# Senpai-sama06/real-time-audio-visual-zooming

Measured on AMD Instinct MI355X. Metric: beamformed TF-bins/sec (2-ch, 1024-pt STFT) + SIR dB delta vs reference, higher is better.
Workload: dtype f32

## Files before the change

### include/avz.h

```cpp
#ifndef AVZ_H_
#define AVZ_H_

#ifdef __cplusplus
extern "C" {
#endif

#define AVZ_OK 0
#define AVZ_ERR_ARG (-1)
#define AVZ_ERR_SHAPE (-2)
#define AVZ_ERR_HIP (-3)
#define AVZ_ERR_UNSUPPORTED (-4)
#define AVZ_ERR_ALIGN (-5)

#define AVZ_MASK_IBM 0
#define AVZ_MASK_IPD 1
#define AVZ_MASK_EXTERNAL 2
#define AVZ_MASK_ONES 3

#define AVZ_PF_NONE 0
#define AVZ_PF_IBM_TARGET 1
#define AVZ_PF_EXT_FLOOR 2
#define AVZ_PF_EXT_MUL 3
#define AVZ_PF_IRM 4

// ... 74 lines not shown
  int batch;
  int frames;
  const float* Y;
  long long y_stride_b, y_stride_m, y_stride_f;
  const float* mask;
  long long mask_stride_b, mask_stride_f;
  const double* steer;
  float* S;
  long long s_stride_b, s_stride_f;
  double* cov_out;
  float* w_out;
  int* fallback;
} avz_spectral_args;
int avz_beamform_spectral(const avz_plan* plan, const avz_spectral_args* args, void* hip_stream);

int avz_istft(const avz_plan* plan, int batch, int frames, const float* S, long long s_stride_b,
              long long s_stride_f, float* out, long long out_stride, float* peak,
              void* workspace, long long workspace_bytes, void* hip_stream);

int avz_plan_set_timing(avz_plan* plan, int enable);
int avz_plan_set_timing_period(avz_plan* plan, int period);
int avz_plan_get_timing(avz_plan* plan, double* ms_avg , int* calls);
int avz_plan_set_ibm_stats(avz_plan* plan, unsigned long long* counts);
int avz_plan_set_diagnostics(avz_plan* plan, int synth_variant, int ipf_mode);
int avz_ibm_window(int n, float* out);

int avz_stft(const avz_plan* plan, int batch, int channels, const int* len, int max_len,
             const float* x, long long x_stride, long long ch_stride, float* Y,
             long long y_stride_b, long long y_stride_c, long long y_stride_f,
             void* hip_stream);

int avz_chunk_split(int n_items, int channels, int chunk, const int* item_utt,
                    const int* item_start, const int* len, const float* x, long long x_stride,
                    long long x_ch_stride, float* items, long long item_stride,
                    long long item_ch_stride, void* hip_stream);

int avz_chunk_merge(int batch, int max_len, int hop, int item_out_len, const int* len,
                    const int* item_base, const float* item_out, long long item_out_stride,
                    float* y, long long y_stride, float* peak, int normalize, double norm_eps,
                    void* hip_stream);

#define AVZ_FEAT_LOGMAG_IPD 1
#define AVZ_FEAT_TFLITE 2
int avz_mask_features(const avz_plan* plan, int layout, int batch, const int* len, int max_len,
                      const float* x, long long x_stride, long long ch_stride, float* feat,
                      long long s_b, long long s_c, long long s_f, long long s_t,
// ... 40 lines not shown
```

### real-time-audio-visual-zooming_amd/avz/_lib.py

```python
from __future__ import annotations

import ctypes as ct
import os

import torch

_HERE = os.path.dirname(os.path.abspath(__file__))
LIB_PATH = os.environ.get("AVZ_LIB", os.path.join(_HERE, "libavz.so"))

AVZ_OK = 0
AVZ_ERR_ARG = -1
AVZ_ERR_SHAPE = -2
AVZ_ERR_HIP = -3
AVZ_ERR_UNSUPPORTED = -4
AVZ_ERR_ALIGN = -5

MASK_IBM, MASK_IPD, MASK_EXTERNAL, MASK_ONES = 0, 1, 2, 3
PF_NONE, PF_IBM_TARGET, PF_EXT_FLOOR, PF_EXT_MUL, PF_IRM = 0, 1, 2, 3, 4
FALLBACK_MIC0, FALLBACK_MEAN, FALLBACK_BATCH = 0, 1, 2
NORM_NONE, NORM_PEAK = 0, 1
BF_MVDR, BF_HYBRID_NULL = 0, 1
FEAT_LOGMAG_IPD, FEAT_TFLITE = 1, 2

EXPORTED = [
    "avz_plan_create", "avz_plan_destroy", "avz_plan_get_config", "avz_num_frames",
    "avz_mvdr_batch", "avz_plan_set_timing", "avz_plan_get_timing", "avz_stft",
    "avz_plan_set_timing_period",
    "avz_chunk_split", "avz_chunk_merge", "avz_mask_features", "avz_srp_scan",
    "avz_projection_metrics", "avz_scene_workspace_bytes", "avz_scene_mix", "avz_strerror",
    "avz_last_hip_error", "avz_version", "avz_mvdr_workspace_bytes",
    "avz_mvdr_covariance", "avz_solve_covariance", "avz_apply_istft", "avz_beamform_spectral",
    "avz_istft", "avz_scene_generate_workspace_bytes", "avz_scene_generate",
    "avz_projection_metrics_scaled", "avz_plan_set_ibm_stats", "avz_plan_set_diagnostics",
    "avz_ibm_window",
]


class AvzConfig(ct.Structure):
    _fields_ = [
        ("fs", ct.c_int), ("n_fft", ct.c_int), ("hop", ct.c_int),
        ("sigma", ct.c_double), ("angle_deg", ct.c_double), ("mic_d", ct.c_double),
        ("c_sound", ct.c_double), ("fmin_hz", ct.c_double),
        ("mask_mode", ct.c_int), ("postfilter", ct.c_int),
        ("pf_floor", ct.c_double), ("weight_eps", ct.c_double),
        ("normalize", ct.c_int), ("norm_eps", ct.c_double),
        ("max_batch", ct.c_int), ("max_samples", ct.c_int),
        ("beamformer", ct.c_int), ("bypass_hz", ct.c_double), ("cond_max", ct.c_double),
        ("singular_fallback", ct.c_int), ("ibm_kappa", ct.c_double),
    ]


class AvzBatchArgs(ct.Structure):
    _fields_ = [
        ("batch", ct.c_int), ("len", ct.c_void_p), ("max_len", ct.c_int),
        ("mix", ct.c_void_p), ("mix_stride", ct.c_longlong), ("ch_stride", ct.c_longlong),
        ("ref_tgt", ct.c_void_p), ("ref_int", ct.c_void_p), ("ref_stride", ct.c_longlong),
        ("ext_mask", ct.c_void_p), ("mask_stride_b", ct.c_longlong),
# ... 48 lines not shown
    lib.avz_plan_create.argtypes = [ct.POINTER(P), ct.POINTER(AvzConfig)]
    lib.avz_plan_destroy.argtypes = [P]
    lib.avz_plan_get_config.argtypes = [P, ct.POINTER(AvzConfig)]
    lib.avz_num_frames.argtypes = [P, ct.c_int]
    lib.avz_mvdr_batch.argtypes = [P, ct.POINTER(AvzBatchArgs), P]
    lib.avz_mvdr_workspace_bytes.argtypes = [P, ct.c_int, ct.c_int]
    lib.avz_mvdr_workspace_bytes.restype = ct.c_longlong
    lib.avz_mvdr_covariance.argtypes = [P, ct.POINTER(AvzBatchArgs), P]
    lib.avz_solve_covariance.argtypes = [P, ct.c_int, P, P, P, P, P]
    lib.avz_apply_istft.argtypes = [P, ct.POINTER(AvzBatchArgs), P, P]
    lib.avz_beamform_spectral.argtypes = [P, ct.POINTER(AvzSpectralArgs), P]
    lib.avz_istft.argtypes = [P, ct.c_int, ct.c_int, P, ct.c_longlong, ct.c_longlong, P,
                              ct.c_longlong, P, P, ct.c_longlong, P]
    for name in ("avz_mvdr_covariance", "avz_solve_covariance", "avz_apply_istft",
                 "avz_beamform_spectral", "avz_istft"):
        getattr(lib, name).restype = ct.c_int
    lib.avz_stft.argtypes = [P, ct.c_int, ct.c_int, P, ct.c_int, P, ct.c_longlong, ct.c_longlong,
                             P, ct.c_longlong, ct.c_longlong, ct.c_longlong, P]
    I, LL = ct.c_int, ct.c_longlong
    lib.avz_plan_set_timing.argtypes = [P, I]
    lib.avz_plan_set_timing_period.argtypes = [P, I]
    lib.avz_plan_get_timing.argtypes = [P, ct.POINTER(ct.c_double), ct.POINTER(I)]
    lib.avz_plan_set_ibm_stats.argtypes = [P, P]
    lib.avz_plan_set_diagnostics.argtypes = [P, I, I]
    lib.avz_ibm_window.argtypes = [I, ct.POINTER(ct.c_float)]
    lib.avz_chunk_split.argtypes = [I, I, I, P, P, P, P, LL, LL, P, LL, LL, P]
    lib.avz_chunk_merge.argtypes = [I, I, I, I, P, P, P, LL, P, LL, P, I, ct.c_double, P]
    lib.avz_mask_features.argtypes = [P, I, I, P, I, P, LL, LL, P, LL, LL, LL, LL, P]
    D = ct.c_double
    lib.avz_srp_scan.argtypes = [P, I, P, I, P, LL, LL, I, D, D, D, D, P, P]
    lib.avz_projection_metrics.argtypes = [I, I, P, P, LL, P, LL, P, LL, P, P, P]
    lib.avz_projection_metrics_scaled.argtypes = [I, I, P, P, LL, P, D, P, LL, P, LL, P, P, P]
    lib.avz_scene_workspace_bytes.argtypes = [I, I, I]
    lib.avz_scene_workspace_bytes.restype = LL
    lib.avz_scene_mix.argtypes = [I, I, I, P, P, P, D, D, D, D, D, P, LL, LL, P, P, LL, P, LL, P]
    lib.avz_scene_generate_workspace_bytes.argtypes = [I, I, I]
    lib.avz_scene_generate_workspace_bytes.restype = LL
    lib.avz_scene_generate.argtypes = [I, LL, I, I, ct.c_uint, D, D, D, D, D, P, LL, LL, P, P, LL,
                                       P, LL, P]
    lib.avz_strerror.argtypes = [ct.c_int]
    lib.avz_strerror.restype = ct.c_char_p
    lib.avz_last_hip_error.restype = ct.c_char_p
    for name in ("avz_plan_create", "avz_plan_destroy", "avz_plan_get_config", "avz_num_frames",
                 "avz_mvdr_batch", "avz_stft", "avz_chunk_split", "avz_chunk_merge",
                 "avz_plan_set_timing", "avz_plan_get_timing", "avz_mask_features",
                 "avz_plan_set_timing_period",
                 "avz_srp_scan", "avz_projection_metrics", "avz_scene_mix",
                 "avz_scene_generate", "avz_projection_metrics_scaled", "avz_version",
                 "avz_plan_set_ibm_stats", "avz_plan_set_diagnostics", "avz_ibm_window"):
        getattr(lib, name).restype = ct.c_int
    if lib.avz_version() != ABI_VERSION:
        raise ImportError(f"libavz ABI version {lib.avz_version()} != {ABI_VERSION} "
                          "(AvzBatchArgs / AvzSpectralArgs layouts); rebuild")
    return lib


lib = _load()


def check(rc: int, what: str) -> int:
    if rc < 0:
        msg = lib.avz_strerror(rc).decode()
        if rc == AVZ_ERR_HIP:
            msg += ": " + lib.avz_last_hip_error().decode()
        raise AvzError(f"{what} failed ({rc}): {msg}")
    return rc
```

### real-time-audio-visual-zooming_amd/avz/engine.py

```python
from __future__ import annotations

import ctypes as ct
from dataclasses import dataclass, field

import torch

from . import _lib
from ._lib import AvzBatchArgs, AvzConfig, check, lib

MASKS = {"ibm": _lib.MASK_IBM, "ipd": _lib.MASK_IPD, "external": _lib.MASK_EXTERNAL,
         "ones": _lib.MASK_ONES}
POSTFILTERS = {"none": _lib.PF_NONE, "ibm": _lib.PF_IBM_TARGET, "floor": _lib.PF_EXT_FLOOR,
               "mul": _lib.PF_EXT_MUL, "irm": _lib.PF_IRM}
FALLBACKS = {"mic0": _lib.FALLBACK_MIC0, "mean": _lib.FALLBACK_MEAN,
             "batch": _lib.FALLBACK_BATCH}
NORMS = {"none": _lib.NORM_NONE, "peak": _lib.NORM_PEAK}
BEAMFORMERS = {"mvdr": _lib.BF_MVDR, "hybrid_null": _lib.BF_HYBRID_NULL}


def n_frames(length: int, hop: int) -> int:
    return -(-length // hop) + 1


def out_length(length: int, hop: int) -> int:
# ... 61 lines not shown
        self._h = h
        self.hop = cfg.n_fft // 2
        self.F = cfg.n_fft // 2 + 1

    def __del__(self):
        h = getattr(self, "_h", None)
        if h is not None and h.value:
            lib.avz_plan_destroy(h)
            self._h = None

    KERNELS = ("analysis", "solve", "synthesis", "finalize")

    def set_timing(self, enable: bool = True, analysis_only: bool = False,
                   period: int = 1) -> None:
        mode = (2 if analysis_only else 1) if enable else 0
        check(lib.avz_plan_set_timing_period(self._h, int(period)), "avz_plan_set_timing_period")
        check(lib.avz_plan_set_timing(self._h, mode), "avz_plan_set_timing")

    def set_ibm_stats(self, counts) -> None:
        if counts is not None:
            assert counts.dtype == torch.int64 and counts.is_cuda and counts.numel() >= 2
        check(lib.avz_plan_set_ibm_stats(self._h, _ptr(counts)), "avz_plan_set_ibm_stats")
        self._ibm_stats = counts

    def set_diagnostics(self, synth_variant: int = 2, ipf_mode: int = 0) -> None:
        check(lib.avz_plan_set_diagnostics(self._h, int(synth_variant), int(ipf_mode)),
              "avz_plan_set_diagnostics")

    def timing(self) -> dict:
        ms = (ct.c_double * 4)()
        n = ct.c_int()
        check(lib.avz_plan_get_timing(self._h, ms, ct.byref(n)), "avz_plan_get_timing")
        return {"calls": n.value, **{k: ms[i] for i, k in enumerate(self.KERNELS)}}

    def frames(self, length: int) -> int:
        return check(lib.avz_num_frames(self._h, int(length)), "avz_num_frames")

    def out_len(self, length: int) -> int:
        return out_length(length, self.hop)

    def alloc_out(self, batch: int, max_len: int, device) -> torch.Tensor:
        n = self.out_len(max_len)
        return torch.empty((batch, (n + 3) // 4 * 4), dtype=torch.float32, device=device)

    def workspace_bytes(self, batch: int, max_len: int) -> int:
        return check(lib.avz_mvdr_workspace_bytes(self._h, int(batch), int(max_len)),
# ... 268 lines not shown
```

### real-time-audio-visual-zooming_amd/csrc/avz_capi.cpp

```cpp
#include <hip/hip_runtime.h>

#include <algorithm>
#include <cmath>
#include <complex>
#include <limits>
#include <cstdlib>
#include <cstring>
#include <new>
#include <string>
#include <vector>

#include "../../include/avz.h"
#include "avz_internal.h"

struct Workspace {
  float* part;
  uint32_t* mwords;
  float* coef;
  float* heads;
  float* tails;
  uint32_t* peak_u;
  int* flag;
  float* pf_gain;
  float* tpart;
// ... 58 lines not shown
    w->xpend = units ? reinterpret_cast<uint32_t*>(q) : nullptr; q += sz_xp;
    w->xdfr = units ? reinterpret_cast<uint32_t*>(q) : nullptr; q += sz_xd;
    w->xunc = units ? reinterpret_cast<uint32_t*>(q) : nullptr; q += sz_xu;
    w->xst = units ? reinterpret_cast<uint32_t*>(q) : nullptr; q += sz_xs;
    w->xst_bytes = sz_xs;
    w->xst_units = units;
    w->xres = units ? reinterpret_cast<float*>(q) : nullptr; q += sz_xr;
  }
  return sz_part + sz_mw + sz_coef + 2 * sz_ht + 6 * sz_b + sz_gain + sz_tpart + 2 * sz_seam +
         sz_xp + sz_xd + sz_xu + sz_xs + sz_xr;
}

struct avz_plan {
  avz_config cfg;
  double tau1, tau2;
  int max_frames;
  int nchunk;
  void* arena;
  double* steer;
  double* xtw;
  float* xwin;
  float ibm_cert;
  unsigned long long* xstat;
  int synth_variant;
  int dbg_ipf;
  Workspace ws;
  bool timing;
  int n_k;
  hipEvent_t ev[2][8];
  bool ev_pending[2];
  int ev_kern[2];
  int ev_next;
  int period;
  long long seen;
  double ms_sum[4];
  int ms_calls;
};

static void timing_drain(avz_plan* p, int set) {
  if (!p->ev_pending[set]) return;
  p->ev_pending[set] = false;
  int last = 0;
  for (int i = 0; i < p->n_k; ++i)
    if ((p->ev_kern[set] >> i) & 1) last = i;
  if (hipEventSynchronize(p->ev[set][2 * last + 1]) != hipSuccess) return;
  for (int i = 0; i < p->n_k; ++i) {
// ... 100 lines not shown
    const size_t sz_tab = sz_steer + sz_xtw + sz_xwin;
    const size_t sz_ws = ws_layout(c, c.max_batch, p->nchunk, nullptr, nullptr);
    hipError_t e = hipMalloc(&p->arena, sz_tab + sz_ws);
    if (e != hipSuccess) {
      delete p;
      return hip_fail(e);
    }
    char* q = static_cast<char*>(p->arena);
    p->steer = reinterpret_cast<double*>(q);
    p->xtw = reinterpret_cast<double*>(q + sz_steer);
    p->xwin = reinterpret_cast<float*>(q + sz_steer + sz_xtw);
    ws_layout(c, c.max_batch, p->nchunk, q + sz_tab, &p->ws);
    if (p->ws.xst) {
      e = hipMemset(p->ws.xst, 0, p->ws.xst_bytes);
      if (e != hipSuccess) {
        (void)hipFree(p->arena);
        delete p;
        return hip_fail(e);
      }
    }
    const double kappa = c.ibm_kappa == 0.0 ? AVZ_IBM_KAPPA : c.ibm_kappa;
    p->ibm_cert = kappa > 0.0 ? (float)(kappa * 0x1p-24) : 0.0f;
    p->xstat = nullptr;
    p->synth_variant = 2;
    p->dbg_ipf = 0;
    std::vector<double> xt((size_t)N * 2);
    for (int j = 0; j < N; ++j) {
      const long double a = -2.0L * 3.141592653589793238462643383279502884L * j / N;
      xt[2 * j] = (double)cosl(a);
      xt[2 * j + 1] = (double)sinl(a);
    }
    std::vector<float> xw((size_t)N);
    ref_window_f32(N, xw.data());
    std::vector<double> st((size_t)F * 4);
    const double df = 1.0 / (c.n_fft * (1.0 / c.fs));
    for (int k = 0; k < F; ++k) {
      const double omega = 2 * M_PI * (k * df);
      const std::complex<double> v0 = std::exp(std::complex<double>(0.0, -omega * p->tau1));
      const std::complex<double> v1 = std::exp(std::complex<double>(0.0, -omega * p->tau2));
      std::complex<double> d0 = v0, d1 = v1;
      if (c.beamformer == AVZ_BF_HYBRID_NULL) {
        const std::complex<double> den = v0 + 1e-10;
        d0 = v0 / den;
        d1 = v1 / den;
      }
      st[4 * k + 0] = d0.real();
// ... 48 lines not shown
static void plan_params(const avz_plan* p, avz::ChainArgs& k) {
  const avz_config& c = p->cfg;
  k.fs = c.fs;
  k.sigma = c.sigma;
  k.tau1 = p->tau1;
  k.tau2 = p->tau2;
  k.mic_d = c.mic_d;
  k.c_sound = c.c_sound;
  k.fmin_hz = c.fmin_hz;
  k.weight_eps = (float)c.weight_eps;
  k.pf_floor = (float)c.pf_floor;
  k.norm_eps = (float)c.norm_eps;
  k.postfilter = c.postfilter;
  k.normalize = c.normalize;
  k.singular_fallback = c.singular_fallback;
  k.beamformer = c.beamformer;
  k.bypass_hz = c.bypass_hz;
  k.cond_max = c.cond_max;
  k.steer = p->steer;
  k.ibm_cert = p->ibm_cert;
  k.xwin = p->xwin;
  k.xtw = p->xtw;
  k.xstat = p->xstat;
  k.synth_variant = p->synth_variant;
  k.dbg_ipf = p->dbg_ipf;
}

enum { USE_CHAIN = 0, USE_COVARIANCE = 1, USE_APPLY = 2 };

static int prepare_chain(const avz_plan* p, const avz_batch_args* a, int use, avz::ChainArgs& k) {
  if (!p || !a) return AVZ_ERR_ARG;
  const avz_config& c = p->cfg;
  if (a->batch < 0 || a->batch > c.max_batch) return AVZ_ERR_SHAPE;
  if (!a->len || !a->mix || (use != USE_COVARIANCE && !a->out)) return AVZ_ERR_ARG;
  if (use == USE_COVARIANCE && !a->cov_out) return AVZ_ERR_ARG;
  if (a->max_len < c.n_fft || a->max_len > c.max_samples) return AVZ_ERR_SHAPE;
  if (a->ch_stride < a->max_len) return AVZ_ERR_SHAPE;
  if (a->batch > 1 && a->mix_stride < a->ch_stride + a->max_len) return AVZ_ERR_SHAPE;
  const int T = frames_for(a->max_len, c.hop);
  const int F = c.n_fft / 2 + 1;
  if (use != USE_COVARIANCE) {
    const long long out_len = (long long)(T - 1) * c.hop;
    if (a->batch > 1 && a->out_stride < out_len) return AVZ_ERR_SHAPE;
    if ((a->out_stride & 3) || (reinterpret_cast<uintptr_t>(a->out) & 15)) return AVZ_ERR_ALIGN;
  }
  if (use != USE_APPLY && c.mask_mode == AVZ_MASK_IBM) {
// ... 231 lines not shown
  if (!enable) return AVZ_OK;
  if (enable != 1 && enable != 2) return AVZ_ERR_ARG;
  p->n_k = enable == 2 ? 1 : 4;
  for (int s = 0; s < 2; ++s)
    for (int i = 0; i < 8; ++i) {
      const hipError_t e = hipEventCreateWithFlags(&p->ev[s][i], hipEventDisableSystemFence);
      if (e != hipSuccess) {
        for (int t = 0; t <= s; ++t)
          for (int j = 0; j < (t < s ? 8 : i); ++j) (void)hipEventDestroy(p->ev[t][j]);
        return hip_fail(e);
      }
    }
  p->timing = true;
  return AVZ_OK;
}

extern "C" int avz_plan_set_ibm_stats(avz_plan* p, unsigned long long* counts) {
  if (!p) return AVZ_ERR_ARG;
  if (misaligned(counts, 8)) return AVZ_ERR_ALIGN;
  p->xstat = counts;
  return AVZ_OK;
}

extern "C" int avz_plan_set_diagnostics(avz_plan* p, int synth_variant, int ipf_mode) {
  if (!p || synth_variant < 0 || synth_variant > 2 || ipf_mode < 0 || ipf_mode > 2)
    return AVZ_ERR_ARG;
  p->synth_variant = synth_variant;
  p->dbg_ipf = ipf_mode;
  return AVZ_OK;
}

extern "C" int avz_plan_set_timing_period(avz_plan* p, int period) {
  if (!p || period < 1) return AVZ_ERR_ARG;
  p->period = period;
  p->seen = 0;
  return AVZ_OK;
}

extern "C" int avz_plan_get_timing(avz_plan* p, double* ms_avg, int* calls) {
  if (!p || !ms_avg) return AVZ_ERR_ARG;
  if (!p->timing) return AVZ_ERR_ARG;
  timing_drain(p, p->ev_next);
  timing_drain(p, p->ev_next ^ 1);
  for (int i = 0; i < 4; ++i)
    ms_avg[i] = i >= p->n_k ? std::numeric_limits<double>::quiet_NaN()
                                 : (p->ms_calls ? p->ms_sum[i] / p->ms_calls : 0.0);
// ... 286 lines not shown
```

### real-time-audio-visual-zooming_amd/csrc/avz_chunked_k.hpp

```cpp
#pragma once
#include <hip/hip_runtime.h>
#include <hip/hip_ext.h>
#include <stdint.h>

#include <algorithm>
#include <atomic>
#include <type_traits>

#include "avz_common.hpp"
#include "avz_ibm_exact.hpp"
#ifndef AVZ_NO_IBM_CERT
#define AVZ_NO_IBM_CERT 0
#endif
#ifndef AVZ_CERT_PARTS
#define AVZ_CERT_PARTS 7
#endif

namespace avz {


constexpr int kChunk = 32;
constexpr int kSC1 = 16;
typedef int v4i_t __attribute__((ext_vector_type(4)));
constexpr int kCThreads = 256;
// ... 309 lines not shown
  return *(KArgs*)u;
}
struct NoTw {};
using Tw1024 = cf[31];
__device__ __forceinline__ int pick(uint32_t packed, int i) {
  return (int)(signed char)(packed >> (8 * i));
}
template <int N>
struct XLds {
  using C = KCfg<N>;
  using X = XGeo<N>;
  static constexpr int FR = 4;
  static constexpr int MP = N / 2 + 4;
  static constexpr int MIC_BYTES = FR / C::FPW * C::WAVE_BYTES;
  static constexpr int MAG_OFF = (4 * X::SCRATCH > MIC_BYTES) ? 4 * X::SCRATCH : MIC_BYTES;
  static constexpr int TWL_OFF = MAG_OFF + 2 * FR * MP * 4;
  static constexpr int WIN_OFF = TWL_OFF + (N / 2) * 16;
  static constexpr int SLOT_OFF = WIN_OFF + N * 4;
  static constexpr int SCAN_OFF = SLOT_OFF + FR * 32;
  static constexpr int SCAN_INTS = 256;
  static constexpr int WL = 32;
  static constexpr int WL_OFF = SCAN_OFF + 256 * 4;
  static constexpr int CTL_OFF = WL_OFF + WL * 16;
  static constexpr int END = CTL_OFF + 32;
  static_assert(C::FPW == 2 && END <= CGeo<N>::SLOT_LDS, "exact phase LDS");
};

struct XSlot {
  int unit, f, e, b, L, c, flags, pad;
};
__device__ __forceinline__ XSlot slot_u(const XSlot* sl, int g) {
  const XSlot v = sl[g];
  XSlot s;
  s.unit = __builtin_amdgcn_readfirstlane(v.unit);
  s.f = __builtin_amdgcn_readfirstlane(v.f);
  s.e = 0;
  s.b = __builtin_amdgcn_readfirstlane(v.b);
  s.L = __builtin_amdgcn_readfirstlane(v.L);
  s.c = __builtin_amdgcn_readfirstlane(v.c);
  s.flags = __builtin_amdgcn_readfirstlane(v.flags);
  s.pad = 0;
  return s;
}
template <int F, class CA>
__device__ __forceinline__ float* unit_item(CA& A, int u, int gx, int n_items, int n_whole, int P,
                                            int& b, int& c) {
  if (u < n_items) {
    b = u / gx;
    c = u % gx;
    return A.part + ((long long)b * A.nchunk + c) * 5 * F;
  }
  const int q = u - n_items, it = n_whole + q / P;
  b = it / gx;
  c = it % gx;
  return A.tpart + (long long)q * 5 * F;
}

template <int N, bool PER_BIN>
__device__ __forceinline__ void exact_round(KArgs& A, unsigned char* lds, const XSlot* sl, int ns,
                                            Acc32 (&pacc)[CGeo<N>::BPT + 1],
                                            uint32_t (&pbits)[CGeo<N>::BPT + 1]) {
  using C = KCfg<N>;
  using G = CGeo<N>;
  using X = XGeo<N>;
  using XL = XLds<N>;
  constexpr int NT = G::NT, H = G::H, F = G::F, BPT = G::BPT, PPL = C::PPL, MP = XL::MP;
  const int tid = threadIdx.x, lane = tid & 63;
  const int wave = __builtin_amdgcn_readfirstlane(tid >> 6);
  float* const mag = reinterpret_cast<float*>(lds + XL::MAG_OFF);
  const cd* const twl = reinterpret_cast<const cd*>(lds + XL::TWL_OFF);
  const float* const win = reinterpret_cast<const float*>(lds + XL::WIN_OFF);
  cd* const buf = reinterpret_cast<cd*>(lds + wave * X::SCRATCH);
  AVZ_STAMP_DECL();
  AVZ_STAMP_INIT();
#ifdef AVZ_XTRACE
  unsigned long long xr_prev = __builtin_amdgcn_s_memrealtime();
#define AVZ_XR(i)                                                                  \
  do {                                                                             \
    if (threadIdx.x == 0 && g_stamps) {                                            \
      const unsigned long long now_ = __builtin_amdgcn_s_memrealtime();            \
      g_stamps[blockIdx.x * 16 + (i)] += now_ - xr_prev;                           \
      xr_prev = now_;                                                              \
    }                                                                              \
  } while (0)
#else
#define AVZ_XR(i) (void)0
#endif
  int lane_o = lane;
  opaque_i(lane_o);
  const int ga = wave >> 1, gb = (wave >> 1) + 2;
  const float* const refp = (wave & 1) ? A.ref_int : A.ref_tgt;
  float xa[N / 64], xb[N / 64];
  if (ga < ns) {
    const XSlot s = slot_u(sl, ga);
    ref_frame_load<N>(make_rsrc(refp + (long long)s.b * A.ref_stride, s.L),
                      (s.c * kChunk + s.f) * H - N / 2, lane_o, xa);
  }
  if (gb < ns) {
    const XSlot s = slot_u(sl, gb);
    ref_frame_load<N>(make_rsrc(refp + (long long)s.b * A.ref_stride, s.L),
                      (s.c * kChunk + s.f) * H - N / 2, lane_o, xb);
  }
  if (ga < ns) ref_spectrum_exact<N>(xa, twl, win, buf, mag + (2 * ga + (wave & 1)) * MP, lane_o);
  AVZ_STAMP(4);
  AVZ_XR(8);
  cf v[PPL];
  LaneMap<N> lm;
  lm.init(lane_o);
  const int gm = C::FPW * wave + lm.grp;
  if (wave < XL::FR / C::FPW) {
    const XSlot s = slot_u(sl, 0);
    const float* mixb = A.mix + (long long)s.b * A.mix_stride;
    const rsrc_t r_m0 = make_rsrc(mixb, s.L), r_m1 = make_rsrc(mixb + A.ch_stride, s.L);
    const bool on = gm < ns;
    const int fm = sl[on ? gm : 0].f;
    const int s0 = (s.c * kChunk + fm) * H - N / 2 + lm.in0;
#pragma unroll
    for (int r = 0; r < PPL; ++r) {
      v[r].x = on ? bload(r_m0, s0 + C::IN_STRIDE * r) : 0.0f;
      v[r].y = on ? bload(r_m1, s0 + C::IN_STRIDE * r) : 0.0f;
    }
  }
  if (gb < ns) {
    int lane_b = lane;
    opaque_i(lane_b);
    ref_spectrum_exact<N>(xb, twl, win, buf, mag + (2 * gb + (wave & 1)) * MP, lane_b);
  }
  AVZ_STAMP(5);
  lds_barrier();
  AVZ_STAMP(6);
  AVZ_XR(9);
  if (wave < XL::FR / C::FPW) {
    WinCoef<N> wc;
    wc.init(lm);
    cf* const spec = slot_ptr<N>(lds, gm);
    if constexpr (N == 1024) {
      Fft1024x2 f;
      f.l = lm.out0;
      window_apply(v, wc.a0, wc.ac, wc.as);
      f.forward(v, spec, reinterpret_cast<const cf*>(lds + G::TW_OFF));
      static_for<0, 32>([&](auto k) { spec[lm.out0 + 32 * k] = v[k]; });
    } else {
      Fft512x2 f;
      f.init(lane_o);
      window_fft<N>(v, wc, f, spec, lm);
    }
  }
  AVZ_STAMP(7);
  lds_barrier();
  AVZ_STAMP(8);
  AVZ_XR(10);
  unsigned long long n_exact = 0;
  for (int g = 0; g < ns; ++g) {
    const XSlot s = slot_u(sl, g);
    const cf* Zm = slot_ptr<N>(lds, g);
    auto put = [&](int j, int k, const Acc32& a, bool dfr, bool noise) {
      if (dfr) {
        pacc[j].c00 += a.c00;
        pacc[j].c11 += a.c11;
        pacc[j].c01r += a.c01r;
        pacc[j].c01i += a.c01i;
        pacc[j].cm += a.cm;
        pbits[j] |= (noise ? 1u : 0u) << s.f;
      }
    };
#pragma unroll
    for (int j = 0; j < BPT; ++j) {
      const int kb = tid + j * NT;
      const int kp = (N - kb) & (N - 1);
      const bool dfr =
          PER_BIN ? ((A.xdfr[(long long)s.unit * F + kb] >> s.f) & 1u)
                  : ((s.flags & 1) &&
                     ((A.xunc[((long long)s.unit * kChunk + s.f) * 32 + (kb & 31)] >> (kb >> 5)) & 1u));
      Acc32 a;
      a.zero();
      bool noise = false;
      if (dfr) {
        noise = mag[(2 * g + 1) * MP + kb] > mag[(2 * g) * MP + kb];
        cf x0, x1;
        split_pair2(Zm[kb], Zm[kp], x0, x1);
        a.add_sel(x0, x1, noise);
        a.cm = noise ? 1.0f : 0.0f;
        n_exact += 1;
      }
      put(j, kb, a, dfr, noise);
    }
    if (tid == NT - 1) {
      const bool dfr = (s.flags >> 1) & 1;
      Acc32 a;
      a.zero();
      bool noise = false;
      if (dfr) {
        noise = mag[(2 * g + 1) * MP + N / 2] > mag[(2 * g) * MP + N / 2];
        cf y0, y1;
        split_pair2(Zm[N / 2], Zm[N / 2], y0, y1);
        const float wn = noise ? 1.0f : 0.0f;
        a.add(y0, y1, wn, wn);
        n_exact += 1;
      }
      put(BPT, N / 2, a, dfr, noise);
    }
  }
  if (A.xstat && n_exact) atomicAdd(A.xstat + 1, n_exact);
  AVZ_STAMP(9);
  lds_barrier();
  AVZ_STAMP(10);
  AVZ_XR(11);
#undef AVZ_XR
}


constexpr int kSparseMax = 12;

constexpr uint32_t kXOpen = 0x80000000u;
constexpr int kXRound = 2;
struct XPieces {
  uint32_t sp;
  int n_sp, nr, npr, n;
};
__device__ __forceinline__ XPieces x_pieces(uint32_t pend, uint32_t big) {
  XPieces q;
  q.sp = pend & ~big;
  q.n_sp = q.sp ? 1 : 0;
  q.nr = (__popc(big) + kXRound - 1) / kXRound;
  q.npr = min(q.nr, kXPieces - q.n_sp);
  q.n = q.n_sp + q.npr;
  return q;
}
__device__ __forceinline__ bool x_has_piece(uint32_t v) {
  return (v & kXOpen) && (v & 0xffffu) < ((v >> 16) & 0xffu);
}

template <int N, int MASK, bool IRM, class TW>
__device__ __forceinline__ void analysis_item(const ChainArgs& A, unsigned char* lds, int c,
                                              int b, int p, int P, int slot, const TW& tw_reg,
                                              const LaneConst<N>& K, int seq) {
  using C = KCfg<N>;
  using G = CGeo<N>;
  constexpr int NT = G::NT, H = G::H, F = G::F, NSLOT = G::NSLOT, BPT = G::BPT, PPL = C::PPL;
  constexpr int FB = (MASK == MASK_IBM) ? NSLOT / 2 : NSLOT;
  static_assert(kChunk % FB == 0, "steps tile the chunk");
  constexpr bool REFBITS = N == 1024 && MASK == MASK_IBM && !IRM && !std::is_same<TW, NoTw>::value;
  constexpr bool SHARE = N == 1024 && MASK != MASK_IPD && !std::is_same<TW, NoTw>::value;
  constexpr bool DLT = MASK == MASK_IBM && !REFBITS;

  const int tid = threadIdx.x;
  const int wave = __builtin_amdgcn_readfirstlane(tid >> 6);
  const int lane = tid & 63;
  const int L = utt_len(A, b);
  if (L < N) return;
  const int T = (L + H - 1) / H + 1;
  const int nch = (T + kChunk - 1) / kChunk;
  if (c >= nch) return;
  if (c == 0 && p == 0 && tid == 0) {
    A.peak_u[b] = 0u;
    if (A.peak && A.normalize != NORM_PEAK) A.peak[b] = 0.0f;
  }
  const int t0 = c * kChunk;
  const int nframes = min(kChunk, T - t0);
  constexpr int SA = kChunk / FB;
  const int s_lo = p * SA / P;
  const int nstep = min((nframes + FB - 1) / FB, (p + 1) * SA / P);
  uint32_t* const pendw = reinterpret_cast<uint32_t*>(lds + G::MISC_OFF + 32 + 12 * (seq & 1));
  if (MASK == MASK_IBM && tid == 0) {
    int z = 0;
    opaque_i(z);
    pendw[0] = (uint32_t)z;
    pendw[1] = (uint32_t)z;
    pendw[2] = (uint32_t)z;
  }

  const typename C::Fft fft = K.fft;
  LaneMap<N> lm;
  {
    int ln = threadIdx.x & 63;
    opaque_i(ln);
// ... 946 lines not shown
    const int k = seq++;
    if (!((mine >> min(k, 31)) & 1u)) return;
    const uint4 rec = reinterpret_cast<const uint4*>(A.xpend)[u];
    if (rec.x == 0u || rec.w != 0u) return;
    if (!have_tables) {
      tables();
      have_tables = true;
    }
    exact_unit<N, PER_BIN>(A, lds, u, gx, n_items, n_whole, P);
  };
  const int n_end = n_whole + (n_items - n_whole) * P;
  for (int u = blockIdx.x; u < n_end; u += gridDim.x) one(u < n_whole ? u : n_items + u - n_whole);
  AVZ_XT(2, __builtin_amdgcn_s_memrealtime());
  {
    const int n_units = n_items + (n_end - n_whole);
    int* const ctl = reinterpret_cast<int*>(lds + XLds<N>::CTL_OFF);
    for (;;) {
#ifdef AVZ_XTRACE
      const unsigned long long tc = __builtin_amdgcn_s_memrealtime();
#endif
      if (tid < 64) {
        const int got = exact_claim(A, n_units, reinterpret_cast<int*>(lds + XLds<N>::SCAN_OFF));
        if (tid == 0) ctl[2] = got;
      }
#ifdef AVZ_XTRACE
      if (tid == 0 && g_stamps) g_stamps[blockIdx.x * 16 + 14] += __builtin_amdgcn_s_memrealtime() - tc;
#endif
      __syncthreads();
      const int got = ctl[2];
      __syncthreads();
      if (got < 0) break;
      if (!have_tables) {
#ifdef AVZ_XTRACE
        const unsigned long long tt = __builtin_amdgcn_s_memrealtime();
#endif
        tables();
        have_tables = true;
#ifdef AVZ_XTRACE
        if (tid == 0 && g_stamps) g_stamps[blockIdx.x * 16 + 15] += __builtin_amdgcn_s_memrealtime() - tt;
#endif
      }
#ifdef AVZ_XTRACE
      const unsigned long long t0x = __builtin_amdgcn_s_memrealtime();
#endif
      exact_piece<N, PER_BIN>(A, lds, got >> 8, got & 0xff, gx, n_items, n_whole, P);
#ifdef AVZ_XTRACE
      if (tid == 0 && g_stamps) {
        unsigned long long* st = g_stamps + blockIdx.x * 16;
        st[4] += 1;
        st[5] += __builtin_amdgcn_s_memrealtime() - t0x;
      }
#endif
    }
  }
  AVZ_XT(3, __builtin_amdgcn_s_memrealtime());
}

template <int N, int MASK, bool IRM, bool SPLIT = false>
__global__ void __launch_bounds__(kCThreads, KCfg<N>::BLOCKS_PER_CU) avz_analysis_kernel(ChainArgs A) {
  using G = CGeo<N>;
  extern __shared__ __align__(16) unsigned char lds[];
  AVZ_XT(0, __builtin_amdgcn_s_memrealtime());
  if (MASK == MASK_IBM && threadIdx.x == 0)
    *reinterpret_cast<uint32_t*>(lds + G::MISC_OFF + 56) = 0u;
// ... 1635 lines not shown
```

### real-time-audio-visual-zooming_amd/csrc/avz_ibm_exact.hpp

```cpp
#pragma once
#include "avz_common.hpp"

namespace avz {

__device__ __forceinline__ float np_abs_c64(float re, float im) {
  const float a = fabsf(re), b = fabsf(im);
  const float l = fmaxf(a, b), s = fminf(a, b);
  if (l == 0.0f) return 0.0f;
  const float r = (float)((double)s / (double)l);
  const float sq = (float)sqrt((double)fmaf(r, r, 1.0f));
  return l * sq;
}

struct cd {
  double x, y;
};
__device__ __forceinline__ cd cd_add(cd a, cd b) { return {a.x + b.x, a.y + b.y}; }
__device__ __forceinline__ cd cd_sub(cd a, cd b) { return {a.x - b.x, a.y - b.y}; }
__device__ __forceinline__ cd cd_mul(cd a, cd b) {
  return {a.x * b.x - a.y * b.y, a.x * b.y + a.y * b.x};
}
__device__ __forceinline__ cd cd_mi(cd a) { return {a.y, -a.x}; }

__device__ __forceinline__ void cd_dft4(cd& a0, cd& a1, cd& a2, cd& a3) {
// ... 45 lines not shown
  for (int j = tid; j < N / 2; j += nt) {
    const double2 w = tw[j];
    twl[j] = {w.x, w.y};
  }
  for (int j = tid; j < N; j += nt) win[j] = xwin[j];
}
template <int N>
__device__ __forceinline__ cd xtw_at(const cd* twl, int j) {
  const cd w = twl[j & (N / 2 - 1)];
  return (j & (N / 2)) ? cd{-w.x, -w.y} : w;
}

template <int N>
__device__ __forceinline__ void ref_frame_load(rsrc_t x, int s0, int lane, float (&xs)[N / 64]) {
#pragma unroll
  for (int r = 0; r < N / 128; ++r) {
    const int n = 2 * (lane + 64 * r);
    xs[2 * r] = bload(x, s0 + n);
    xs[2 * r + 1] = bload(x, s0 + n + 1);
  }
}

template <int N>
__device__ __forceinline__ void ref_spectrum_exact(const float (&xs)[N / 64], const cd* twl,
                                                   const float* win, cd* buf, float* mag,
                                                   int lane) {
  using X = XGeo<N>;
  constexpr int M = X::M, RX = X::RX;
  cd v[RX];
#pragma unroll
  for (int r = 0; r < RX; ++r) {
    const float2 w = reinterpret_cast<const float2*>(win)[lane + 64 * r];
    v[r] = {(double)w.x * (double)xs[2 * r], (double)w.y * (double)xs[2 * r + 1]};
  }
  int Ns = 1;
#pragma unroll
  for (int p = 0; p < X::PASSES; ++p) {
    const int j = lane;
    const int k = j & (Ns - 1);
    if (p > 0) {
      cd w[RX];
#pragma unroll
      for (int r = 1; r < RX; ++r) w[r] = xtw_at<N>(twl, (r * k * (N / (Ns * RX))) & (N - 1));
#pragma unroll
      for (int r = 0; r < RX; ++r) v[r] = buf[j + r * (M / RX)];
#pragma unroll
      for (int r = 1; r < RX; ++r) v[r] = cd_mul(v[r], w[r]);
    }
    cd_dft<RX>(v);
    __builtin_amdgcn_wave_barrier();
    __builtin_amdgcn_fence(__ATOMIC_RELEASE, "wavefront");
#pragma unroll
    for (int r = 0; r < RX; ++r) buf[(j - k) * RX + k + r * Ns] = v[r];
    __builtin_amdgcn_fence(__ATOMIC_ACQUIRE, "wavefront");
    __builtin_amdgcn_wave_barrier();
    Ns *= RX;
  }
#pragma unroll
  for (int q = 0; q < RX; ++q) {
    const int k = lane + 64 * q;
    const cd zk = buf[k], zm = buf[(M - k) & (M - 1)];
    const cd w = twl[k];
    float re, im;
    if (k == 0) {
      re = (float)(zk.x + zk.y);
      im = 0.0f;
    } else {
      const cd e = {0.5 * (zk.x + zm.x), 0.5 * (zk.y - zm.y)};
      const cd o = {0.5 * (zk.y + zm.y), 0.5 * (zm.x - zk.x)};
      const cd xo = cd_mul(w, o);
      re = (float)(e.x + xo.x);
      im = (float)(e.y + xo.y);
    }
    mag[k] = np_abs_c64(re, im);
    if (k == 0) mag[M] = np_abs_c64((float)(zk.x - zk.y), 0.0f);
  }
}

}
```

### real-time-audio-visual-zooming_amd/csrc/avz_internal.h

```cpp
#pragma once
#include <stdint.h>

namespace avz {

enum : int { MASK_IBM = 0, MASK_IPD = 1, MASK_EXTERNAL = 2, MASK_ONES = 3 };
enum : int { PF_NONE = 0, PF_IBM_TARGET = 1, PF_EXT_FLOOR = 2, PF_EXT_MUL = 3, PF_IRM = 4 };
enum : int { NORM_NONE = 0, NORM_PEAK = 1 };

enum : int { BF_MVDR = 0, BF_HYBRID_NULL = 1 };

struct PieceState {
  uint32_t cnt, fin;
  unsigned long long st;
};
static_assert(sizeof(PieceState) == 16, "one 16-B store resets it");

constexpr int kXPieces = 8;

struct ChainArgs {
  int batch;
  const int* len;
  int max_len;
  const float* mix;
  long long mix_stride;
// ... 25 lines not shown
  uint32_t* peak_u;
  float* pf_gain;
  int singular_fallback;
  const float* spec;
  long long spec_sb, spec_sf;
  int spec_frames;
  int cov_only;
  int* flag;
  int a_whole, a_pieces;
  float* tpart;
  int tpart_slots;
  int s_whole, s_pieces, s_steps;
  float* pheads;
  float* ptails;
  int pseam_slots;
  int b_lo;
  int s_ipf;
  PieceState* pstate;
  int dbg_ipf;
  float ibm_cert;
  const float* xwin;
  const double* xtw;
  unsigned long long* xstat;
  uint32_t* xpend;
  uint32_t* xdfr;
  uint32_t* xunc;
  uint32_t* xst;
  float* xres;
  uint32_t* xhint;
  long long xst_reset;
  int synth_variant;
  void* const* events;
  int n_events;
};

struct SpecArgs {
  int batch, frames;
  const float* Y;
  long long y_sb, y_sm, y_sf;
  const float* M;
  long long m_sb, m_sf;
  const double* steer;
  float* S;
  long long s_sb, s_sf;
  double* cov_out;
  float* w_out;
// ... 102 lines not shown
```

Before: 80.07 billion.

## Skip quiet-reference exact spectra in IBM path using L1 bound gate

Adds a quiet-frame gate to the exact IBM reference phase. The windowed L1 norm of each reference frame bounds every spectral magnitude, so when one source is far quieter than the other the mask decision is fixed and only the louder source's spectrum is computed, with a fallback recompute if any deferred bin falls below the bound. When both gated frames are quiet the mic FFT overlaps with the reference transform on a spare wave. The change also fills twiddle tables while the work claim runs, and clears pending flags for early-exit blocks. It adds LDS usage, extra barriers and branching, and a conservative correctness check that may trigger recomputation.

```diff
diff --git a/include/avz.h b/include/avz.h
--- a/include/avz.h
+++ b/include/avz.h
@@ -120,6 +120,7 @@
 int avz_plan_set_timing_period(avz_plan* plan, int period);
 int avz_plan_get_timing(avz_plan* plan, double* ms_avg , int* calls);
 int avz_plan_set_ibm_stats(avz_plan* plan, unsigned long long* counts);
+int avz_plan_set_ibm_quiet(avz_plan* plan, int enable, unsigned long long* counts );
 int avz_plan_set_diagnostics(avz_plan* plan, int synth_variant, int ipf_mode);
 int avz_ibm_window(int n, float* out);
 
diff --git a/real-time-audio-visual-zooming_amd/avz/_lib.py b/real-time-audio-visual-zooming_amd/avz/_lib.py
--- a/real-time-audio-visual-zooming_amd/avz/_lib.py
+++ b/real-time-audio-visual-zooming_amd/avz/_lib.py
@@ -32,7 +32,7 @@
     "avz_mvdr_covariance", "avz_solve_covariance", "avz_apply_istft", "avz_beamform_spectral",
     "avz_istft", "avz_scene_generate_workspace_bytes", "avz_scene_generate",
     "avz_projection_metrics_scaled", "avz_plan_set_ibm_stats", "avz_plan_set_diagnostics",
-    "avz_ibm_window",
+    "avz_ibm_window", "avz_plan_set_ibm_quiet",
 ]
 
 
@@ -127,6 +127,7 @@
     lib.avz_plan_set_timing_period.argtypes = [P, I]
     lib.avz_plan_get_timing.argtypes = [P, ct.POINTER(ct.c_double), ct.POINTER(I)]
     lib.avz_plan_set_ibm_stats.argtypes = [P, P]
+    lib.avz_plan_set_ibm_quiet.argtypes = [P, I, P]
     lib.avz_plan_set_diagnostics.argtypes = [P, I, I]
     lib.avz_ibm_window.argtypes = [I, ct.POINTER(ct.c_float)]
     lib.avz_chunk_split.argtypes = [I, I, I, P, P, P, P, LL, LL, P, LL, LL, P]
@@ -152,7 +153,8 @@
                  "avz_plan_set_timing_period",
                  "avz_srp_scan", "avz_projection_metrics", "avz_scene_mix",
                  "avz_scene_generate", "avz_projection_metrics_scaled", "avz_version",
-                 "avz_plan_set_ibm_stats", "avz_plan_set_diagnostics", "avz_ibm_window"):
+                 "avz_plan_set_ibm_stats", "avz_plan_set_ibm_quiet", "avz_plan_set_diagnostics",
+                 "avz_ibm_window"):
         getattr(lib, name).restype = ct.c_int
     if lib.avz_version() != ABI_VERSION:
         raise ImportError(f"libavz ABI version {lib.avz_version()} != {ABI_VERSION} "
diff --git a/real-time-audio-visual-zooming_amd/avz/engine.py b/real-time-audio-visual-zooming_amd/avz/engine.py
--- a/real-time-audio-visual-zooming_amd/avz/engine.py
+++ b/real-time-audio-visual-zooming_amd/avz/engine.py
@@ -107,6 +107,13 @@
             assert counts.dtype == torch.int64 and counts.is_cuda and counts.numel() >= 2
         check(lib.avz_plan_set_ibm_stats(self._h, _ptr(counts)), "avz_plan_set_ibm_stats")
         self._ibm_stats = counts
+
+    def set_ibm_quiet(self, enable: bool = True, counts=None) -> None:
+        if counts is not None:
+            assert counts.dtype == torch.int64 and counts.is_cuda and counts.numel() >= 2
+        check(lib.avz_plan_set_ibm_quiet(self._h, int(bool(enable)), _ptr(counts)),
+              "avz_plan_set_ibm_quiet")
+        self._ibm_quiet_counts = counts
 
     def set_diagnostics(self, synth_variant: int = 2, ipf_mode: int = 0) -> None:
         check(lib.avz_plan_set_diagnostics(self._h, int(synth_variant), int(ipf_mode)),
diff --git a/real-time-audio-visual-zooming_amd/csrc/avz_capi.cpp b/real-time-audio-visual-zooming_amd/csrc/avz_capi.cpp
--- a/real-time-audio-visual-zooming_amd/csrc/avz_capi.cpp
+++ b/real-time-audio-visual-zooming_amd/csrc/avz_capi.cpp
@@ -104,6 +104,8 @@
   float* xwin;
   float ibm_cert;
   unsigned long long* xstat;
+  int ibm_quiet;
+  unsigned long long* xqstat;
   int synth_variant;
   int dbg_ipf;
   Workspace ws;
@@ -250,6 +252,8 @@
     const double kappa = c.ibm_kappa == 0.0 ? AVZ_IBM_KAPPA : c.ibm_kappa;
     p->ibm_cert = kappa > 0.0 ? (float)(kappa * 0x1p-24) : 0.0f;
     p->xstat = nullptr;
+    p->ibm_quiet = 1;
+    p->xqstat = nullptr;
     p->synth_variant = 2;
     p->dbg_ipf = 0;
     std::vector<double> xt((size_t)N * 2);
@@ -344,6 +348,8 @@
   k.xwin = p->xwin;
   k.xtw = p->xtw;
   k.xstat = p->xstat;
+  k.ibm_quiet = p->ibm_quiet;
+  k.xqstat = p->xqstat;
   k.synth_variant = p->synth_variant;
   k.dbg_ipf = p->dbg_ipf;
 }
@@ -621,6 +627,14 @@
   return AVZ_OK;
 }
 
+extern "C" int avz_plan_set_ibm_quiet(avz_plan* p, int enable, unsigned long long* counts) {
+  if (!p) return AVZ_ERR_ARG;
+  if (misaligned(counts, 8)) return AVZ_ERR_ALIGN;
+  p->ibm_quiet = enable ? 1 : 0;
+  p->xqstat = counts;
+  return AVZ_OK;
+}
+
 extern "C" int avz_plan_set_diagnostics(avz_plan* p, int synth_variant, int ipf_mode) {
   if (!p || synth_variant < 0 || synth_variant > 2 || ipf_mode < 0 || ipf_mode > 2)
     return AVZ_ERR_ARG;
diff --git a/real-time-audio-visual-zooming_amd/csrc/avz_chunked_k.hpp b/real-time-audio-visual-zooming_amd/csrc/avz_chunked_k.hpp
--- a/real-time-audio-visual-zooming_amd/csrc/avz_chunked_k.hpp
+++ b/real-time-audio-visual-zooming_amd/csrc/avz_chunked_k.hpp
@@ -355,8 +355,12 @@
   static constexpr int WL = 32;
   static constexpr int WL_OFF = SCAN_OFF + 256 * 4;
   static constexpr int CTL_OFF = WL_OFF + WL * 16;
-  static constexpr int END = CTL_OFF + 32;
-  static_assert(C::FPW == 2 && END <= CGeo<N>::SLOT_LDS, "exact phase LDS");
+  static constexpr int QT_OFF = CTL_OFF + 32;
+  static constexpr int END = QT_OFF + FR * 16 + FR * 4;
+  static constexpr int OVL_BUF_OFF = C::WAVE_BYTES;
+  static_assert(C::FPW == 2 && END <= CGeo<N>::SLOT_LDS && QT_OFF % 8 == 0 &&
+                    OVL_BUF_OFF % 16 == 0 && OVL_BUF_OFF + 2 * X::SCRATCH <= MAG_OFF,
+                "exact phase LDS");
 };
 
 struct XSlot {
@@ -403,7 +407,7 @@
   float* const mag = reinterpret_cast<float*>(lds + XL::MAG_OFF);
   const cd* const twl = reinterpret_cast<const cd*>(lds + XL::TWL_OFF);
   const float* const win = reinterpret_cast<const float*>(lds + XL::WIN_OFF);
-  cd* const buf = reinterpret_cast<cd*>(lds + wave * X::SCRATCH);
+  cd* buf = reinterpret_cast<cd*>(lds + wave * X::SCRATCH);
   AVZ_STAMP_DECL();
   AVZ_STAMP_INIT();
 #ifdef AVZ_XTRACE
@@ -421,27 +425,62 @@
 #endif
   int lane_o = lane;
   opaque_i(lane_o);
+  double* const l1s = reinterpret_cast<double*>(lds + XL::QT_OFF);
+  int* const qfail = reinterpret_cast<int*>(lds + XL::QT_OFF + XL::FR * 16);
+  const bool quiet_on = A.ibm_quiet != 0;
+  struct QGate {
+    bool open, loud_int;
+    float ub;
+  };
+  auto gate = [&](int g) {
+    QGate r{false, false, 0.0f};
+    if (quiet_on) {
+      const double lt = l1s[2 * g], li = l1s[2 * g + 1];
+      const bool loud_int = li > lt;
+      const double q = loud_int ? lt : li, l = loud_int ? li : lt;
+      r.open = __builtin_amdgcn_readfirstlane((int)(q <= 0x1p-24 * l)) != 0;
+      r.loud_int = __builtin_amdgcn_readfirstlane((int)loud_int) != 0;
+      r.ub = ref_quiet_ub<N>(q);
+    }
+    return r;
+  };
+  constexpr bool OVL = !PER_BIN && N == 1024;
+  const bool may_ovl = OVL && quiet_on && ns <= 2;
   const int ga = wave >> 1, gb = (wave >> 1) + 2;
   const float* const refp = (wave & 1) ? A.ref_int : A.ref_tgt;
   float xa[N / 64], xb[N / 64];
+  uint32_t dma = 0u, dmb = 0u;
+  bool nyqa = false, nyqb = false;
+  auto deferred_bins = [&](const XSlot& s, uint32_t& dm, bool& nyq) {
+    nyq = (s.flags >> 1) & 1;
+    if constexpr (PER_BIN) {
+#pragma unroll
+      for (int q = 0; q < X::RX; ++q)
+        dm |= ((A.xdfr[(long long)s.unit * F + lane_o + 64 * q] >> s.f) & 1u) << q;
+    } else if (s.flags & 1) {
+      const uint32_t w = A.xunc[((long long)s.unit * kChunk + s.f) * 32 + (lane_o & 31)];
+#pragma unroll
+      for (int q = 0; q < X::RX; ++q) dm |= ((w >> ((lane_o >> 5) + 2 * q)) & 1u) << q;
+    }
+  };
+  auto ref_load = [&](int g, float(&x)[N / 64]) {
+    const XSlot s = slot_u(sl, g);
+    ref_frame_load<N>(make_rsrc(refp + (long long)s.b * A.ref_stride, s.L),
+                      (s.c * kChunk + s.f) * H - N / 2, lane_o, x);
+  };
   if (ga < ns) {
-    const XSlot s = slot_u(sl, ga);
-    ref_frame_load<N>(make_rsrc(refp + (long long)s.b * A.ref_stride, s.L),
-                      (s.c * kChunk + s.f) * H - N / 2, lane_o, xa);
+    ref_load(ga, xa);
+    if (quiet_on) deferred_bins(slot_u(sl, ga), dma, nyqa);
   }
   if (gb < ns) {
-    const XSlot s = slot_u(sl, gb);
-    ref_frame_load<N>(make_rsrc(refp + (long long)s.b * A.ref_stride, s.L),
-                      (s.c * kChunk + s.f) * H - N / 2, lane_o, xb);
-  }
-  if (ga < ns) ref_spectrum_exact<N>(xa, twl, win, buf, mag + (2 * ga + (wave & 1)) * MP, lane_o);
-  AVZ_STAMP(4);
-  AVZ_XR(8);
+    ref_load(gb, xb);
+    if (quiet_on) deferred_bins(slot_u(sl, gb), dmb, nyqb);
+  }
   cf v[PPL];
   LaneMap<N> lm;
   lm.init(lane_o);
-  const int gm = C::FPW * wave + lm.grp;
-  if (wave < XL::FR / C::FPW) {
+  int gm = C::FPW * wave + lm.grp;
+  auto mic_loads = [&]() {
     const XSlot s = slot_u(sl, 0);
     const float* mixb = A.mix + (long long)s.b * A.mix_stride;
     const rsrc_t r_m0 = make_rsrc(mixb, s.L), r_m1 = make_rsrc(mixb + A.ch_stride, s.L);
@@ -453,17 +492,8 @@
       v[r].x = on ? bload(r_m0, s0 + C::IN_STRIDE * r) : 0.0f;
       v[r].y = on ? bload(r_m1, s0 + C::IN_STRIDE * r) : 0.0f;
     }
-  }
-  if (gb < ns) {
-    int lane_b = lane;
-    opaque_i(lane_b);
-    ref_spectrum_exact<N>(xb, twl, win, buf, mag + (2 * gb + (wave & 1)) * MP, lane_b);
-  }
-  AVZ_STAMP(5);
-  lds_barrier();
-  AVZ_STAMP(6);
-  AVZ_XR(9);
-  if (wave < XL::FR / C::FPW) {
+  };
+  auto mic_fft = [&]() {
     WinCoef<N> wc;
     wc.init(lm);
     cf* const spec = slot_ptr<N>(lds, gm);
@@ -478,15 +508,90 @@
       f.init(lane_o);
       window_fft<N>(v, wc, f, spec, lm);
     }
-  }
-  AVZ_STAMP(7);
+  };
+  if (quiet_on) {
+    if (tid < XL::FR) qfail[tid] = 0;
+    if (ga < ns) {
+      const double l1 = ref_frame_l1<N>(xa, win, lane_o);
+      if (lane == 0) l1s[2 * ga + (wave & 1)] = l1;
+    }
+    if (gb < ns) {
+      const double l1 = ref_frame_l1<N>(xb, win, lane_o);
+      if (lane == 0) l1s[2 * gb + (wave & 1)] = l1;
+    }
+    lds_barrier();
+  }
+  bool ovl = false;
+  int mic_wave = 0;
+  if (may_ovl) {
+    const QGate q0 = gate(0), q1 = ns > 1 ? gate(1) : q0;
+    ovl = q0.open && q1.open;
+    mic_wave = q0.loud_int ? 0 : 1;
+  }
+  if (ovl) {
+    buf = reinterpret_cast<cd*>(lds + XL::OVL_BUF_OFF + ga * X::SCRATCH);
+    gm = lm.grp;
+  }
+  const bool mic = ovl ? wave == mic_wave : wave < XL::FR / C::FPW;
+  auto my_turn = [&](int g, int pass, QGate& q) {
+    q = gate(g);
+    const bool quiet = q.open && ((wave & 1) != 0) != q.loud_int;
+    return pass == 0 ? !quiet : quiet && __builtin_amdgcn_readfirstlane(qfail[g]) != 0;
+  };
+  auto transform = [&](int g, int pass, const float(&x)[N / 64], int ln, uint32_t dm, bool nyq) {
+    QGate q;
+    if (g < ns && my_turn(g, pass, q)) {
+      const bool chk = pass == 0 && q.open;
+      const bool below = ref_spectrum_exact<N, true>(x, twl, win, buf, mag + (2 * g + (wave & 1)) * MP,
+                                                     ln, q.ub, chk ? dm : 0u, chk && nyq);
+      if (below && lane == 0) qfail[g] = 1;
+    }
+  };
+  constexpr bool MIC_EARLY = PER_BIN;
+  transform(ga, 0, xa, lane_o, dma, nyqa);
+  AVZ_STAMP(4);
+  AVZ_XR(8);
+  if (MIC_EARLY && mic) mic_loads();
+  {
+    int lane_b = lane;
+    opaque_i(lane_b);
+    transform(gb, 0, xb, lane_b, dmb, nyqb);
+  }
+  if (!MIC_EARLY && mic) mic_loads();
+  if (ovl && mic) mic_fft();
+  AVZ_STAMP(5);
   lds_barrier();
+  if (quiet_on &&
+      __builtin_amdgcn_readfirstlane(qfail[0] | qfail[1] | qfail[2] | qfail[3]) != 0) {
+    QGate q;
+    float xc[N / 64];
+    if (ga < ns && my_turn(ga, 1, q)) {
+      ref_load(ga, xc);
+      transform(ga, 1, xc, lane_o, 0u, false);
+    }
+    if (gb < ns && my_turn(gb, 1, q)) {
+      ref_load(gb, xc);
+      transform(gb, 1, xc, lane_o, 0u, false);
+    }
+    lds_barrier();
+  }
+  AVZ_STAMP(6);
+  AVZ_XR(9);
+  if (!ovl) {
+    if (mic) mic_fft();
+    AVZ_STAMP(7);
+    lds_barrier();
+  }
   AVZ_STAMP(8);
   AVZ_XR(10);
   unsigned long long n_exact = 0;
+  unsigned long long n_one = 0, n_both = 0;
   for (int g = 0; g < ns; ++g) {
     const XSlot s = slot_u(sl, g);
     const cf* Zm = slot_ptr<N>(lds, g);
+    const QGate qg = gate(g);
+    const bool one = qg.open && __builtin_amdgcn_readfirstlane(qfail[g]) == 0;
+    if (qg.open) (one ? n_one : n_both) += 1;
     auto put = [&](int j, int k, const Acc32& a, bool dfr, bool noise) {
       if (dfr) {
         pacc[j].c00 += a.c00;
@@ -509,7 +614,7 @@
       a.zero();
       bool noise = false;
       if (dfr) {
-        noise = mag[(2 * g + 1) * MP + kb] > mag[(2 * g) * MP + kb];
+        noise = one ? qg.loud_int : mag[(2 * g + 1) * MP + kb] > mag[(2 * g) * MP + kb];
         cf x0, x1;
         split_pair2(Zm[kb], Zm[kp], x0, x1);
         a.add_sel(x0, x1, noise);
@@ -524,7 +629,8 @@
       a.zero();
       bool noise = false;
       if (dfr) {
-        noise = mag[(2 * g + 1) * MP + N / 2] > mag[(2 * g) * MP + N / 2];
+        noise = one ? qg.loud_int
+                    : mag[(2 * g + 1) * MP + N / 2] > mag[(2 * g) * MP + N / 2];
         cf y0, y1;
         split_pair2(Zm[N / 2], Zm[N / 2], y0, y1);
         const float wn = noise ? 1.0f : 0.0f;
@@ -535,6 +641,10 @@
     }
   }
   if (A.xstat && n_exact) atomicAdd(A.xstat + 1, n_exact);
+  if (A.xqstat && tid == 0) {
+    if (n_one) atomicAdd(A.xqstat, n_one);
+    if (n_both) atomicAdd(A.xqstat + 1, n_both);
+  }
   AVZ_STAMP(9);
   lds_barrier();
   AVZ_STAMP(10);
@@ -581,10 +691,16 @@
   const int wave = __builtin_amdgcn_readfirstlane(tid >> 6);
   const int lane = tid & 63;
   const int L = utt_len(A, b);
-  if (L < N) return;
   const int T = (L + H - 1) / H + 1;
   const int nch = (T + kChunk - 1) / kChunk;
-  if (c >= nch) return;
+  if (L < N || c >= nch) {
+    if (MASK == MASK_IBM && tid == 0 && A.xpend) {
+      const int gxi = (A.max_frames + kChunk - 1) / kChunk;
+      const int unit = slot < 0 ? b * gxi + c : gxi * A.batch + slot;
+      A.xpend[4 * (long long)unit] = 0u;
+    }
+    return;
+  }
   if (c == 0 && p == 0 && tid == 0) {
     A.peak_u[b] = 0u;
     if (A.peak && A.normalize != NORM_PEAK) A.peak[b] = 0.0f;
@@ -1577,7 +1693,13 @@
       if (tid < 64) {
         const int got = exact_claim(A, n_units, reinterpret_cast<int*>(lds + XLds<N>::SCAN_OFF));
         if (tid == 0) ctl[2] = got;
-      }
+      } else if (!have_tables) {
+        int t = threadIdx.x - 64;
+        opaque_i(t);
+        xtab_fill<N>(A.xtw, A.xwin, reinterpret_cast<cd*>(lds + XL::TWL_OFF),
+                     reinterpret_cast<float*>(lds + XL::WIN_OFF), t, G::NT - 64);
+      }
+      have_tables = true;
 #ifdef AVZ_XTRACE
       if (tid == 0 && g_stamps) g_stamps[blockIdx.x * 16 + 14] += __builtin_amdgcn_s_memrealtime() - tc;
 #endif
@@ -1585,16 +1707,6 @@
       const int got = ctl[2];
       __syncthreads();
       if (got < 0) break;
-      if (!have_tables) {
-#ifdef AVZ_XTRACE
-        const unsigned long long tt = __builtin_amdgcn_s_memrealtime();
-#endif
-        tables();
-        have_tables = true;
-#ifdef AVZ_XTRACE
-        if (tid == 0 && g_stamps) g_stamps[blockIdx.x * 16 + 15] += __builtin_amdgcn_s_memrealtime() - tt;
-#endif
-      }
 #ifdef AVZ_XTRACE
       const unsigned long long t0x = __builtin_amdgcn_s_memrealtime();
 #endif
diff --git a/real-time-audio-visual-zooming_amd/csrc/avz_ibm_exact.hpp b/real-time-audio-visual-zooming_amd/csrc/avz_ibm_exact.hpp
--- a/real-time-audio-visual-zooming_amd/csrc/avz_ibm_exact.hpp
+++ b/real-time-audio-visual-zooming_amd/csrc/avz_ibm_exact.hpp
@@ -91,9 +91,31 @@
 }
 
 template <int N>
-__device__ __forceinline__ void ref_spectrum_exact(const float (&xs)[N / 64], const cd* twl,
+__device__ __forceinline__ double ref_frame_l1(const float (&xs)[N / 64], const float* win,
+                                               int lane) {
+  double s = 0.0;
+#pragma unroll
+  for (int r = 0; r < N / 128; ++r) {
+    const float2 w = reinterpret_cast<const float2*>(win)[lane + 64 * r];
+    s += fabs((double)w.x * (double)xs[2 * r]) + fabs((double)w.y * (double)xs[2 * r + 1]);
+  }
+#pragma unroll
+  for (int o = 32; o > 0; o >>= 1) s += __shfl_xor(s, o, 64);
+  return s;
+}
+template <int N>
+__device__ __forceinline__ float ref_quiet_ub(double l1) {
+  const double t = l1 * (1.0 + 0x1p-18) + 0x1p-148;
+  float f = (float)t;
+  if ((double)f < t) f = __uint_as_float(__float_as_uint(f) + 1u);
+  return f;
+}
+
+template <int N, bool CHECK = false>
+__device__ __forceinline__ bool ref_spectrum_exact(const float (&xs)[N / 64], const cd* twl,
                                                    const float* win, cd* buf, float* mag,
-                                                   int lane) {
+                                                   int lane, float ub = 0.0f, uint32_t dm = 0u,
+                                                   bool nyq = false) {
   using X = XGeo<N>;
   constexpr int M = X::M, RX = X::RX;
   cd v[RX];
@@ -125,6 +147,7 @@
     __builtin_amdgcn_wave_barrier();
     Ns *= RX;
   }
+  bool below = false;
 #pragma unroll
   for (int q = 0; q < RX; ++q) {
     const int k = lane + 64 * q;
@@ -141,9 +164,16 @@
       re = (float)(e.x + xo.x);
       im = (float)(e.y + xo.y);
     }
-    mag[k] = np_abs_c64(re, im);
-    if (k == 0) mag[M] = np_abs_c64((float)(zk.x - zk.y), 0.0f);
+    const float m = np_abs_c64(re, im);
+    mag[k] = m;
+    if (CHECK && ((dm >> q) & 1u) && !(m > ub)) below = true;
+    if (k == 0) {
+      const float mn = np_abs_c64((float)(zk.x - zk.y), 0.0f);
+      mag[M] = mn;
+      if (CHECK && nyq && !(mn > ub)) below = true;
+    }
   }
+  return CHECK && __ballot(below) != 0ull;
 }
 
 }
diff --git a/real-time-audio-visual-zooming_amd/csrc/avz_internal.h b/real-time-audio-visual-zooming_amd/csrc/avz_internal.h
--- a/real-time-audio-visual-zooming_amd/csrc/avz_internal.h
+++ b/real-time-audio-visual-zooming_amd/csrc/avz_internal.h
@@ -71,6 +71,8 @@
   const float* xwin;
   const double* xtw;
   unsigned long long* xstat;
+  int ibm_quiet;
+  unsigned long long* xqstat;
   uint32_t* xpend;
   uint32_t* xdfr;
   uint32_t* xunc;
```

New measurement: 79.19 billion. 1.1% lower.
